# alexkroman/tiny-audio

Hardware: AMD Instinct MI355X
Metric: training audio-sec/sec on 10s@16kHz clips (higher is better)
Workload: dtype bf16

## Files before the change

tiny_audio_amd/csrc/attention_enc.hip:

```cpp
#include <cstdlib>
#include <type_traits>
#include "common.h"
#include "../../include/ta355.h"

namespace {
constexpr int HD = 64;
constexpr int KT = 64;
constexpr int TILE = KT * HD * 2;
constexpr float NEG_BIG = -1.0e30f;
constexpr float RESCALE_THR = 8.0f;

__device__ __forceinline__ int kswz(int r) { return (r >> 1) & 7; }
__device__ __forceinline__ int vswz(int r) { return ((r >> 1) & 3) << 1; }

__device__ __forceinline__ void dma16(const void* g, unsigned lds) {
  asm volatile("s_mov_b32 m0, %0\n\ts_nop 0\n\tglobal_load_lds_dwordx4 %1, off" ::"s"(lds), "v"(g) : "memory");
}

__device__ __forceinline__ bool decode_group(int id, int gsz, int ngroups, int& group, int& member) {
  const int xcd = id & 7, w = id >> 3;
  member = w % gsz;
  group = (w / gsz) * 8 + xcd;
  return group < ngroups;
}
inline int grouped_grid(int gsz, int ngroups) { return gsz * ((ngroups + 7) / 8 * 8); }

__device__ __forceinline__ float max3(float a, float b, float c) { return __builtin_fmaxf(__builtin_fmaxf(a, b), c); }
__device__ __forceinline__ float group_max(float x) {
  auto r = __builtin_amdgcn_permlane16_swap(__float_as_uint(x), __float_as_uint(x), false, false);
  x = fmaxf(__uint_as_float(r[0]), __uint_as_float(r[1]));
  auto q = __builtin_amdgcn_permlane32_swap(__float_as_uint(x), __float_as_uint(x), false, false);
  return fmaxf(__uint_as_float(q[0]), __uint_as_float(q[1]));
}
__device__ __forceinline__ bf16x8 pack_p(const f32x4& a, const f32x4& b) {
  union { bf16x8 v; uint32_t u[4]; } r;
  r.u[0] = pack2bf(a[0], a[1]); r.u[1] = pack2bf(a[2], a[3]);
  r.u[2] = pack2bf(b[0], b[1]); r.u[3] = pack2bf(b[2], b[3]);
  return r.v;
}
typedef __attribute__((ext_vector_type(4))) short bf16x4_t;
__device__ __forceinline__ bf16x8 read_vfrag_tr(const char* vt, int dt, int l15, int c0, int c1) {
  const int dcol = dt * 16 + 4 * (l15 & 3);
  const int chunk = dcol >> 3, half = (dcol >> 2) & 1;
  const int r0 = c0 + (l15 >> 2), r1 = c1 + (l15 >> 2);
  const bf16x4_t a = __builtin_amdgcn_ds_read_tr16_b64_v4i16(
      (__attribute__((address_space(3))) bf16x4_t*)(vt + r0 * 128 + ((chunk ^ vswz(r0)) << 4) + half * 8));
  const bf16x4_t b = __builtin_amdgcn_ds_read_tr16_b64_v4i16(
      (__attribute__((address_space(3))) bf16x4_t*)(vt + r1 * 128 + ((chunk ^ vswz(r1)) << 4) + half * 8));
  return (bf16x8){a[0], a[1], a[2], a[3], b[0], b[1], b[2], b[3]};
}

template <int QSUB>
__global__ __launch_bounds__(256) void attn_enc_fwd_kernel(const bf16_t* __restrict__ qkv, bf16_t* __restrict__ O, int B, int NH,
                                                           int L, long rs) {
  __shared__ __attribute__((aligned(16))) char smem[4 * TILE];
  const int tid = threadIdx.x, lane = tid & 63, wave = tid >> 6, g = lane >> 4, l15 = lane & 15;
  constexpr int QROWS = 64 * QSUB;
  const int nq = (L + QROWS - 1) / QROWS;
  int group, qt;
  if (!decode_group(blockIdx.x, nq, B * NH, group, qt)) return;
  const int b = group / NH, h = group % NH;
  const int q0 = qt * QROWS + wave * 16 * QSUB;
  const int Hd = NH * HD;
  const bf16_t* Qb = qkv + (long)b * L * rs + h * HD;
  const bf16_t* Kb = Qb + Hd;
  const int ntiles = (L + KT - 1) / KT;

  const unsigned lds0 = __builtin_amdgcn_readfirstlane((unsigned)(unsigned long)(__attribute__((address_space(3))) char*)smem + wave * 2048);
  const bf16_t* src[4];
#pragma unroll
  for (int i = 0; i < 2; ++i) {
    const int r = (wave * 2 + i) * 8 + (lane >> 3);
    src[i] = Kb + (long)r * rs + (((lane & 7) ^ kswz(r)) << 3);
    src[2 + i] = Kb + Hd + (long)r * rs + (((lane & 7) ^ vswz(r)) << 3);
  }
  const long tstride = (long)KT * rs;
  auto dma = [&](int t, int buf) {
    const unsigned dst = lds0 + buf * (2 * TILE);
    if ((t + 1) * KT <= L) {
      dma16(src[0], dst); dma16(src[2], dst + TILE); dma16(src[1], dst + 1024); dma16(src[3], dst + TILE + 1024);
    } else {
#pragma unroll
      for (int i = 0; i < 2; ++i) {
        const int key = t * KT + (wave * 2 + i) * 8 + (lane >> 3);
        const long back = key < L ? 0 : (long)(L - 1 - key) * rs;
        dma16(src[i] + back, dst + i * 1024); dma16(src[2 + i] + back, dst + TILE + i * 1024);
      }
    }
#pragma unroll
    for (int j = 0; j < 4; ++j) src[j] += tstride;
  };
  dma(0, 0);

  bf16x8 qf[QSUB][2];
#pragma unroll
  for (int sub = 0; sub < QSUB; ++sub) {
    int qr = q0 + sub * 16 + l15; qr = qr < L ? qr : L - 1;
#pragma unroll
    for (int ks = 0; ks < 2; ++ks) qf[sub][ks] = *(const bf16x8*)(Qb + (long)qr * rs + ks * 32 + g * 8);
  }
  f32x4 o[QSUB][5];
  f32x4 negm[QSUB];
#pragma unroll
  for (int sub = 0; sub < QSUB; ++sub) {
#pragma unroll
    for (int i = 0; i < 5; ++i) o[sub][i] = (f32x4){0.f, 0.f, 0.f, 0.f};
    negm[sub] = (f32x4){0.f, 0.f, 0.f, 0.f};
  }
  const bf16x8 ones = {0x3f80, 0x3f80, 0x3f80, 0x3f80, 0x3f80, 0x3f80, 0x3f80, 0x3f80};

  auto tile = [&](const int t, auto masked_tag) {
    constexpr bool MASKED = decltype(masked_tag)::value;
    const char* Ks = smem + (t & 1) * (2 * TILE);
    const char* Vs = Ks + TILE;
    asm volatile("s_waitcnt vmcnt(0)" ::: "memory");
    __syncthreads();
    if (t + 1 < ntiles) dma(t + 1, (t + 1) & 1);
    f32x4 s[QSUB][4];
#pragma unroll
    for (int kt = 0; kt < 4; ++kt) {
      const int kr = kt * 16 + l15;
      const bf16x8 a0 = *(const bf16x8*)(Ks + kr * 128 + (((0 + g) ^ kswz(kr)) << 4));
      const bf16x8 a1 = *(const bf16x8*)(Ks + kr * 128 + (((4 + g) ^ kswz(kr)) << 4));
#pragma unroll
      for (int sub = 0; sub < QSUB; ++sub) {
        s[sub][kt] = __builtin_amdgcn_mfma_f32_16x16x32_bf16(a0, qf[sub][0], negm[sub], 0, 0, 0);
        s[sub][kt] = __builtin_amdgcn_mfma_f32_16x16x32_bf16(a1, qf[sub][1], s[sub][kt], 0, 0, 0);
      }
    }
#pragma unroll
    for (int sub = 0; sub < QSUB; ++sub) {
      if constexpr (MASKED) {
#pragma unroll
        for (int kt = 0; kt < 4; ++kt)
#pragma unroll
          for (int r = 0; r < 4; ++r)
            if (t * KT + kt * 16 + g * 4 + r >= L) s[sub][kt][r] = NEG_BIG;
      }
      float mx = max3(s[sub][0][0], s[sub][0][1], s[sub][0][2]);
      mx = max3(mx, s[sub][0][3], s[sub][1][0]);
      mx = max3(mx, s[sub][1][1], s[sub][1][2]);
      mx = max3(mx, s[sub][1][3], s[sub][2][0]);
      mx = max3(mx, s[sub][2][1], s[sub][2][2]);
      mx = max3(mx, s[sub][2][3], s[sub][3][0]);
      mx = max3(mx, s[sub][3][1], s[sub][3][2]);
      mx = fmaxf(mx, s[sub][3][3]);
      mx = group_max(mx);
      if (t == 0 || __any(mx > RESCALE_THR)) {
        const float d = t == 0 ? mx : fmaxf(mx, 0.f);
        const float alpha = __builtin_amdgcn_exp2f(-d);
#pragma unroll
        for (int i = 0; i < 5; ++i) { o[sub][i][0] *= alpha; o[sub][i][1] *= alpha; o[sub][i][2] *= alpha; o[sub][i][3] *= alpha; }
#pragma unroll
        for (int kt = 0; kt < 4; ++kt) { s[sub][kt][0] -= d; s[sub][kt][1] -= d; s[sub][kt][2] -= d; s[sub][kt][3] -= d; }
        negm[sub][0] -= d; negm[sub][1] -= d; negm[sub][2] -= d; negm[sub][3] -= d;
      }
#pragma unroll
      for (int kt = 0; kt < 4; ++kt)
#pragma unroll
        for (int r = 0; r < 4; ++r) s[sub][kt][r] = __builtin_amdgcn_exp2f(s[sub][kt][r]);
    }
#pragma unroll
    for (int kp = 0; kp < 2; ++kp) {
      bf16x8 pb[QSUB];
#pragma unroll
      for (int sub = 0; sub < QSUB; ++sub) pb[sub] = pack_p(s[sub][2 * kp], s[sub][2 * kp + 1]);
#pragma unroll
      for (int dt = 0; dt < 4; ++dt) {
        const bf16x8 va = read_vfrag_tr(Vs, dt, l15, (2 * kp) * 16 + g * 4, (2 * kp + 1) * 16 + g * 4);
#pragma unroll
        for (int sub = 0; sub < QSUB; ++sub) o[sub][dt] = __builtin_amdgcn_mfma_f32_16x16x32_bf16(va, pb[sub], o[sub][dt], 0, 0, 0);
      }
#pragma unroll
      for (int sub = 0; sub < QSUB; ++sub) o[sub][4] = __builtin_amdgcn_mfma_f32_16x16x32_bf16(ones, pb[sub], o[sub][4], 0, 0, 0);
    }
  };
  const int nfull = L / KT;
  for (int t = 0; t < nfull; ++t) tile(t, std::false_type{});
  for (int t = nfull; t < ntiles; ++t) tile(t, std::true_type{});

  __syncthreads();
  char* stage = smem + wave * (QSUB * 2048);
#pragma unroll
  for (int sub = 0; sub < QSUB; ++sub) {
    const float inv = 1.0f / o[sub][4][0];
    const int row = sub * 16 + l15;
#pragma unroll
    for (int dt = 0; dt < 4; ++dt) {
      uint2 w;
      w.x = pack2bf(o[sub][dt][0] * inv, o[sub][dt][1] * inv);
      w.y = pack2bf(o[sub][dt][2] * inv, o[sub][dt][3] * inv);
      const int chunk = dt * 2 + (g >> 1);
      *(uint2*)(stage + row * 128 + ((chunk ^ kswz(row)) << 4) + (g & 1) * 8) = w;
    }
  }
#pragma unroll
  for (int i = 0; i < QSUB * 2; ++i) {
    const int row = i * 8 + (lane >> 3), p = lane & 7;
    const uint4 v = *(const uint4*)(stage + row * 128 + ((p ^ kswz(row)) << 4));
    const int qrow = q0 + row;
    if (qrow < L) *(uint4*)(O + ((long)b * L + qrow) * Hd + h * HD + p * 8) = v;
  }
}
}

extern "C" int ta_attention_enc_fwd(const void* qkv, void* out, int B, int heads, int S, hipStream_t st) {
  if (B <= 0 || heads <= 0 || S <= 0) return TA_ERR_ARG;
  const long rs = 3L * heads * HD;
  constexpr int QSUB = 2;
  const int nq = (S + 64 * QSUB - 1) / (64 * QSUB);
  TA_LAUNCH((attn_enc_fwd_kernel<QSUB>), dim3(grouped_grid(nq, B * heads)), dim3(256), 0, st, (const bf16_t*)qkv, (bf16_t*)out, B,
            heads, S, rs);
  TA_CHECK_LAUNCH();
  return TA_OK;
}
```

Measured before the change: 7696.

## Trim encoder attention registers with SGPR-base DMA, peeled first tile, and staged epilogue

Replaces the four per-lane 64-bit DMA source pointers with 32-bit per-lane offsets plus one scalar base that advances per tile. It also makes the wave index uniform, sets launch bounds to four blocks per CU, and peels the first tile so the t==0 rescale branch disappears from the steady-state loop. The epilogue now stages output into the idle K/V buffer without a trailing __syncthreads, and the first DMA is issued after the Q loads. Compile-time-gated timestamp instrumentation is added but off by default. The main risks are 32-bit offset overflow for very large row strides, and register spills or an unsynchronised buffer reuse from the new occupancy bound.

```diff
diff --git a/tiny_audio_amd/csrc/attention_enc.hip b/tiny_audio_amd/csrc/attention_enc.hip
--- a/tiny_audio_amd/csrc/attention_enc.hip
+++ b/tiny_audio_amd/csrc/attention_enc.hip
@@ -10,11 +10,25 @@
 constexpr float NEG_BIG = -1.0e30f;
 constexpr float RESCALE_THR = 8.0f;
 
+#ifdef TA355_ATTN_ENC_STAMPS
+constexpr int ENC_STAMP_SLOTS = 48, ENC_STAMP_TILES = 10, ENC_STAMP_WGS = 2560;
+__device__ unsigned g_enc_stamps[ENC_STAMP_WGS * 4 * ENC_STAMP_SLOTS];
+#define ENC_STAMP_VAL(i, val) do { __builtin_amdgcn_sched_barrier(0); \
+    if ((i) >= 0 && (i) < ENC_STAMP_SLOTS && (threadIdx.x & 63) == 0) stamp_lds[(threadIdx.x >> 6) * ENC_STAMP_SLOTS + (i)] = (unsigned)(val); \
+    __builtin_amdgcn_sched_barrier(0); } while (0)
+#define ENC_STAMP(i) ENC_STAMP_VAL(i, __builtin_amdgcn_s_memtime())
+#define ENC_STAMP_TILE(t, k) ENC_STAMP((t) < ENC_STAMP_TILES ? 8 + 4 * (t) + (k) : -1)
+#else
+#define ENC_STAMP_VAL(i, val) do { } while (0)
+#define ENC_STAMP(i) do { } while (0)
+#define ENC_STAMP_TILE(t, k) do { } while (0)
+#endif
+
 __device__ __forceinline__ int kswz(int r) { return (r >> 1) & 7; }
 __device__ __forceinline__ int vswz(int r) { return ((r >> 1) & 3) << 1; }
 
-__device__ __forceinline__ void dma16(const void* g, unsigned lds) {
-  asm volatile("s_mov_b32 m0, %0\n\ts_nop 0\n\tglobal_load_lds_dwordx4 %1, off" ::"s"(lds), "v"(g) : "memory");
+__device__ __forceinline__ void dma16(const void* base, unsigned off, unsigned lds) {
+  asm volatile("s_mov_b32 m0, %0\n\ts_nop 0\n\tglobal_load_lds_dwordx4 %1, %2" ::"s"(lds), "v"(off), "s"(base) : "memory");
 }
 
 __device__ __forceinline__ bool decode_group(int id, int gsz, int ngroups, int& group, int& member) {
@@ -51,10 +65,18 @@
 }
 
 template <int QSUB>
-__global__ __launch_bounds__(256) void attn_enc_fwd_kernel(const bf16_t* __restrict__ qkv, bf16_t* __restrict__ O, int B, int NH,
+__global__ __launch_bounds__(256, 4) void attn_enc_fwd_kernel(const bf16_t* __restrict__ qkv, bf16_t* __restrict__ O, int B, int NH,
                                                            int L, long rs) {
   __shared__ __attribute__((aligned(16))) char smem[4 * TILE];
-  const int tid = threadIdx.x, lane = tid & 63, wave = tid >> 6, g = lane >> 4, l15 = lane & 15;
+#ifdef TA355_ATTN_ENC_STAMPS
+  __shared__ unsigned stamp_lds[4 * ENC_STAMP_SLOTS];
+  for (int i = threadIdx.x; i < 4 * ENC_STAMP_SLOTS; i += 256) stamp_lds[i] = 0;
+  __syncthreads();
+  ENC_STAMP(0);
+  ENC_STAMP_VAL(4, __builtin_amdgcn_s_memrealtime());
+#endif
+  const int tid = threadIdx.x, lane = tid & 63, g = lane >> 4, l15 = lane & 15;
+  const int wave = __builtin_amdgcn_readfirstlane(tid >> 6);
   constexpr int QROWS = 64 * QSUB;
   const int nq = (L + QROWS - 1) / QROWS;
   int group, qt;
@@ -66,32 +88,32 @@
   const bf16_t* Kb = Qb + Hd;
   const int ntiles = (L + KT - 1) / KT;
 
-  const unsigned lds0 = __builtin_amdgcn_readfirstlane((unsigned)(unsigned long)(__attribute__((address_space(3))) char*)smem + wave * 2048);
-  const bf16_t* src[4];
+  const unsigned lds0 = __builtin_amdgcn_readfirstlane((unsigned)(unsigned long)(__attribute__((address_space(3))) char*)smem) + wave * 2048;
+  const unsigned rsb = (unsigned)rs * 2;
+  unsigned soff[4];
 #pragma unroll
   for (int i = 0; i < 2; ++i) {
     const int r = (wave * 2 + i) * 8 + (lane >> 3);
-    src[i] = Kb + (long)r * rs + (((lane & 7) ^ kswz(r)) << 3);
-    src[2 + i] = Kb + Hd + (long)r * rs + (((lane & 7) ^ vswz(r)) << 3);
-  }
+    soff[i] = r * rsb + (((lane & 7) ^ kswz(r)) << 4);
+    soff[2 + i] = r * rsb + Hd * 2 + (((lane & 7) ^ vswz(r)) << 4);
+  }
+  const bf16_t* kt_base = Kb;
   const long tstride = (long)KT * rs;
   auto dma = [&](int t, int buf) {
     const unsigned dst = lds0 + buf * (2 * TILE);
     if ((t + 1) * KT <= L) {
-      dma16(src[0], dst); dma16(src[2], dst + TILE); dma16(src[1], dst + 1024); dma16(src[3], dst + TILE + 1024);
+      dma16(kt_base, soff[0], dst); dma16(kt_base, soff[2], dst + TILE);
+      dma16(kt_base, soff[1], dst + 1024); dma16(kt_base, soff[3], dst + TILE + 1024);
     } else {
 #pragma unroll
       for (int i = 0; i < 2; ++i) {
         const int key = t * KT + (wave * 2 + i) * 8 + (lane >> 3);
-        const long back = key < L ? 0 : (long)(L - 1 - key) * rs;
-        dma16(src[i] + back, dst + i * 1024); dma16(src[2 + i] + back, dst + TILE + i * 1024);
-      }
-    }
-#pragma unroll
-    for (int j = 0; j < 4; ++j) src[j] += tstride;
+        const unsigned back = key < L ? 0u : (unsigned)(key - (L - 1)) * rsb;
+        dma16(kt_base, soff[i] - back, dst + i * 1024); dma16(kt_base, soff[2 + i] - back, dst + TILE + i * 1024);
+      }
+    }
+    kt_base += tstride;
   };
-  dma(0, 0);
-
   bf16x8 qf[QSUB][2];
 #pragma unroll
   for (int sub = 0; sub < QSUB; ++sub) {
@@ -99,6 +121,8 @@
 #pragma unroll
     for (int ks = 0; ks < 2; ++ks) qf[sub][ks] = *(const bf16x8*)(Qb + (long)qr * rs + ks * 32 + g * 8);
   }
+  asm volatile("" ::: "memory");
+  dma(0, 0);
   f32x4 o[QSUB][5];
   f32x4 negm[QSUB];
 #pragma unroll
@@ -109,12 +133,14 @@
   }
   const bf16x8 ones = {0x3f80, 0x3f80, 0x3f80, 0x3f80, 0x3f80, 0x3f80, 0x3f80, 0x3f80};
 
-  auto tile = [&](const int t, auto masked_tag) {
-    constexpr bool MASKED = decltype(masked_tag)::value;
+  auto tile = [&](const int t, auto first_tag, auto masked_tag) {
+    constexpr bool FIRST = decltype(first_tag)::value, MASKED = decltype(masked_tag)::value;
     const char* Ks = smem + (t & 1) * (2 * TILE);
     const char* Vs = Ks + TILE;
     asm volatile("s_waitcnt vmcnt(0)" ::: "memory");
+    if constexpr (FIRST) ENC_STAMP(1);
     __syncthreads();
+    ENC_STAMP_TILE(t, 0);
     if (t + 1 < ntiles) dma(t + 1, (t + 1) & 1);
     f32x4 s[QSUB][4];
 #pragma unroll
@@ -128,6 +154,7 @@
         s[sub][kt] = __builtin_amdgcn_mfma_f32_16x16x32_bf16(a1, qf[sub][1], s[sub][kt], 0, 0, 0);
       }
     }
+    ENC_STAMP_TILE(t, 1);
 #pragma unroll
     for (int sub = 0; sub < QSUB; ++sub) {
       if constexpr (MASKED) {
@@ -146,8 +173,12 @@
       mx = max3(mx, s[sub][3][1], s[sub][3][2]);
       mx = fmaxf(mx, s[sub][3][3]);
       mx = group_max(mx);
-      if (t == 0 || __any(mx > RESCALE_THR)) {
-        const float d = t == 0 ? mx : fmaxf(mx, 0.f);
+      if constexpr (FIRST) {
+#pragma unroll
+        for (int kt = 0; kt < 4; ++kt) { s[sub][kt][0] -= mx; s[sub][kt][1] -= mx; s[sub][kt][2] -= mx; s[sub][kt][3] -= mx; }
+        negm[sub][0] -= mx; negm[sub][1] -= mx; negm[sub][2] -= mx; negm[sub][3] -= mx;
+      } else if (__any(mx > RESCALE_THR)) {
+        const float d = fmaxf(mx, 0.f);
         const float alpha = __builtin_amdgcn_exp2f(-d);
 #pragma unroll
         for (int i = 0; i < 5; ++i) { o[sub][i][0] *= alpha; o[sub][i][1] *= alpha; o[sub][i][2] *= alpha; o[sub][i][3] *= alpha; }
@@ -160,6 +191,7 @@
 #pragma unroll
         for (int r = 0; r < 4; ++r) s[sub][kt][r] = __builtin_amdgcn_exp2f(s[sub][kt][r]);
     }
+    ENC_STAMP_TILE(t, 2);
 #pragma unroll
     for (int kp = 0; kp < 2; ++kp) {
       bf16x8 pb[QSUB];
@@ -174,35 +206,58 @@
 #pragma unroll
       for (int sub = 0; sub < QSUB; ++sub) o[sub][4] = __builtin_amdgcn_mfma_f32_16x16x32_bf16(ones, pb[sub], o[sub][4], 0, 0, 0);
     }
+    ENC_STAMP_TILE(t, 3);
   };
   const int nfull = L / KT;
-  for (int t = 0; t < nfull; ++t) tile(t, std::false_type{});
-  for (int t = nfull; t < ntiles; ++t) tile(t, std::true_type{});
-
-  __syncthreads();
-  char* stage = smem + wave * (QSUB * 2048);
+  if (nfull > 0) tile(0, std::true_type{}, std::false_type{}); else tile(0, std::true_type{}, std::true_type{});
+  for (int t = 1; t < nfull; ++t) tile(t, std::false_type{}, std::false_type{});
+  for (int t = nfull > 0 ? nfull : 1; t < ntiles; ++t) tile(t, std::false_type{}, std::true_type{});
+
+  static_assert(4 * QSUB * 2048 <= 2 * TILE, "the four waves' output rows fit one K | V buffer");
+  ENC_STAMP(2);
+  int lane_o = lane;
+  asm volatile("" : "+v"(lane_o));
+  const int g_o = lane_o >> 4, l15_o = lane_o & 15;
+  char* stage = smem + (ntiles & 1) * (2 * TILE) + wave * (QSUB * 2048);
 #pragma unroll
   for (int sub = 0; sub < QSUB; ++sub) {
     const float inv = 1.0f / o[sub][4][0];
-    const int row = sub * 16 + l15;
+    const int row = sub * 16 + l15_o;
 #pragma unroll
     for (int dt = 0; dt < 4; ++dt) {
       uint2 w;
       w.x = pack2bf(o[sub][dt][0] * inv, o[sub][dt][1] * inv);
       w.y = pack2bf(o[sub][dt][2] * inv, o[sub][dt][3] * inv);
-      const int chunk = dt * 2 + (g >> 1);
-      *(uint2*)(stage + row * 128 + ((chunk ^ kswz(row)) << 4) + (g & 1) * 8) = w;
+      const int chunk = dt * 2 + (g_o >> 1);
+      *(uint2*)(stage + row * 128 + ((chunk ^ kswz(row)) << 4) + (g_o & 1) * 8) = w;
     }
   }
 #pragma unroll
   for (int i = 0; i < QSUB * 2; ++i) {
-    const int row = i * 8 + (lane >> 3), p = lane & 7;
+    const int row = i * 8 + (lane_o >> 3), p = lane_o & 7;
     const uint4 v = *(const uint4*)(stage + row * 128 + ((p ^ kswz(row)) << 4));
     const int qrow = q0 + row;
     if (qrow < L) *(uint4*)(O + ((long)b * L + qrow) * Hd + h * HD + p * 8) = v;
   }
-}
-}
+#ifdef TA355_ATTN_ENC_STAMPS
+  ENC_STAMP(3);
+  ENC_STAMP_VAL(5, __builtin_amdgcn_s_memrealtime());
+  ENC_STAMP_VAL(6, (__builtin_amdgcn_s_getreg(((16 - 1) << 11) | (0 << 6) | 4) & 0xffff) |
+                       (__builtin_amdgcn_s_getreg(((4 - 1) << 11) | (0 << 6) | 20) << 16));
+  ENC_STAMP_VAL(7, ntiles);
+  asm volatile("s_waitcnt lgkmcnt(0)" ::: "memory");
+  if (blockIdx.x < ENC_STAMP_WGS && lane < ENC_STAMP_SLOTS)
+    g_enc_stamps[((long)blockIdx.x * 4 + wave) * ENC_STAMP_SLOTS + lane] = stamp_lds[wave * ENC_STAMP_SLOTS + lane];
+#endif
+}
+}
+
+#ifdef TA355_ATTN_ENC_STAMPS
+extern "C" int ta_debug_attn_enc_stamps(unsigned* host_out, int nwaves) {
+  if (nwaves < 0 || nwaves > ENC_STAMP_WGS * 4) return TA_ERR_ARG;
+  return hipMemcpyFromSymbol(host_out, HIP_SYMBOL(g_enc_stamps), (size_t)nwaves * ENC_STAMP_SLOTS * sizeof(unsigned)) == hipSuccess ? TA_OK : 2;
+}
+#endif
 
 extern "C" int ta_attention_enc_fwd(const void* qkv, void* out, int B, int heads, int S, hipStream_t st) {
   if (B <= 0 || heads <= 0 || S <= 0) return TA_ERR_ARG;
```

Measured after the change: 7697, median of 2. Within noise of the previous version (+0.0%).
